# philgzl/brever

Measured on AMD Instinct MI355X. Metric: utterances/sec (4 s @16 kHz) Conv-TasNet train, higher is better.
Workload: dtype bf16

## Files before the change

### brever_amd/csrc/bwd_fused.cuh

```cuda
#pragma once
#include "tcn_kernels.cuh"

namespace brv {

#ifndef BF_ABL
#define BF_ABL 0
#endif

#ifndef BF_AHEAD1
#define BF_AHEAD1 4
#endif
#ifndef BF_AHEAD2
#define BF_AHEAD2 4
#endif
#ifndef BF_PIPE
#define BF_PIPE 1
#endif

struct BwdFusedParams {
  DwParams d;
  const bf16_t* g;
  int ldg, Kg;
  const bf16_t* Wp;
  const float* gamma2;
  float* dgamma2; float* dbeta2;
  int K, R;
#ifdef BF_STAMP
  long long* dbg;
#endif
};

#ifndef BF_ROWS_N
#define BF_ROWS_N 256
#endif
#ifndef BF_WPS
#define BF_WPS 3
#endif
constexpr int BF_ROWS = BF_ROWS_N;
constexpr int BF_LDW = HL_CG + 8;
constexpr int BF_LDS = BF_ROWS*BF_LDW*2 + 32*HL_CG*4;

inline void bf_tile_shape(int T, int dil, int P, int& K, int& R) {
  const int n_teeth = (T - 1)/dil + 1;
  long long best = -1;
  K = 1; R = 1;
  for (int r = 1; r <= HL_RMAX*2 && r <= dil; ++r) {
    const int kmax = BF_ROWS/r - (P - 1);
    if (kmax < 1) break;
    const int n_qt = ceil_div(n_teeth, kmax);
    const int k = ceil_div(n_teeth, n_qt);
    const long long tiles = (long long)n_qt*ceil_div(dil, r);
    const long long cost = tiles*100000 + tiles*(k + P - 1)*r;
    if (best < 0 || cost <= best) { best = cost; K = k; R = r; }
  }
}

#ifdef BF_STAMP
#define BF_MARK(i) do { long long t_; asm volatile("s_memtime %0\n\ts_waitcnt lgkmcnt(0)" : "=s"(t_) :: "memory"); \
                        if (threadIdx.x == 0 && fp.dbg) fp.dbg[(long long)blockIdx.x*8 + (i)] = t_; } while (0)
#else
#define BF_MARK(i) do { } while (0)
#endif
constexpr int kRowBad = 1 << 21;
constexpr int kRowCentre = 1 << 30;
constexpr int kRowFrame = kRowCentre - 1;
inline bool bf_frames_ok(long long T) { return T < kRowBad; }

template <int P, int KG>
__global__ __launch_bounds__(256, BF_WPS) void dwconv_bwd_fused_kernel(const BwdFusedParams fp) {
  const DwParams& p = fp.d;
  extern __shared__ __attribute__((aligned(16))) unsigned char dyn_lds[];
  bf16_t* win = reinterpret_cast<bf16_t*>(dyn_lds);
  float* red = reinterpret_cast<float*>(dyn_lds + BF_ROWS*BF_LDW*2);
  const int tid = threadIdx.x, lane = tid & 63, wid = tid >> 6;
  const int T = p.T, d = p.dil;
  const int R = fp.R, K = fp.K;
  const int n_rt = ceil_div(d, R);
  const int n_teeth = (T - 1)/d + 1;
  const int n_qt = ceil_div(n_teeth, K);
  const int n_tt = n_rt*n_qt, n_cg = p.Cp/HL_CG;
  const int xcd = blockIdx.x & 7, slot = blockIdx.x >> 3;
  const int cg = slot % n_cg;
  const int id = (slot / n_cg)*8 + xcd;
  if (id >= n_tt*p.B) return;
  const int b = id / n_tt;
  const int tile = id % n_tt;
  const int r0 = (tile % n_rt)*R, q0 = (tile / n_rt)*K;
  BF_MARK(0);
  const int cl = (tid & 7)*8;
  const int c0 = cg*HL_CG + cl;
  const int rslot = tid >> 3;
  const int W = (K + P - 1)*R;
  const int KR = K*R;
  const int qbase = q0 - (P - 1) + p.left/d;
  __shared__ int wtab[BF_ROWS];
  __shared__ int otab[BF_ROWS];
  {
    int qi, ri;
    if ((R & (R - 1)) == 0) { ri = tid & (R - 1); qi = tid >> (31 - __builtin_clz(R)); }
    else {
      qi = (int)(((float)tid + 0.5f)*(1.f/(float)R)); ri = tid - qi*R;
    }
    const int q = qbase + qi;
    const int tf = q*d + r0 + ri;
    const bool in = tid < W && q >= 0 && r0 + ri < d && tf < T;
    wtab[tid] = in ? (tf | ((q >= q0 && q < q0 + K) ? kRowCentre : 0)) : kRowBad;
    const int to = (q0 + qi)*d + r0 + ri;
    otab[tid] = (tid < KR && r0 + ri < d && to < T) ? to : kRowBad;
  }
  __shared__ float ptab[(3 + P)*HL_CG];
  float pv0 = 0.f, pv1 = 0.f;
  auto ptab_src = [&](int idx) -> const float* {
    const int which = idx >> 6, c = cg*HL_CG + (idx & 63);
    return which == 0 ? fp.gamma2 + c : which == 1 ? p.gamma1 + c : which == 2 ? p.beta1 + c
                      : p.taps + (long long)c*P + (which - 3);
  };
  {
    const float* s0 = ptab_src(tid);
    if (s0) pv0 = *s0;
    if (tid + 256 < (3 + P)*HL_CG) { const float* s1 = ptab_src(tid + 256); if (s1) pv1 = *s1; }
  }
  asm volatile("s_waitcnt lgkmcnt(0)\n\ts_barrier" ::: "memory");

  const __amdgpu_buffer_rsrc_t rz2 = make_rsrc(p.z2in + (long long)b*T*p.Cp, (long long)T*p.Cp*2);
  const __amdgpu_buffer_rsrc_t rz1 = make_rsrc(p.z1 + (long long)b*T*p.Cp, (long long)T*p.Cp*2);
  const unsigned int row = (unsigned int)(p.Cp*2), coff = (unsigned int)(c0*2);
  auto row_off = [&](int v) { return __umul24((unsigned int)(v & kRowFrame), row) + coff; };
  uint4 qzA[4], qz1A[4];
  {
    const int n32 = lane & 31, h = lane >> 5;
    const int oct = lane & 7, rsub = lane >> 3;
    const int widu = __builtin_amdgcn_readfirstlane(wid);
    const int ngrp = (W + 31) >> 5;
    const bool act0 = 2*widu < ngrp, act1 = 2*widu + 1 < ngrp;
    const __amdgpu_buffer_rsrc_t rg =
        make_rsrc(fp.g + (long long)b*T*fp.ldg, ((long long)(T - 1)*fp.ldg + KG)*2);
    unsigned int offG[8];
#pragma unroll
    for (int i = 0; i < 8; ++i)
      offG[i] = __umul24((unsigned int)(wtab[64*widu + 8*i + rsub] & kRowFrame), (unsigned int)(fp.ldg*2)) + (unsigned int)(oct*16);
    constexpr int nkc = KG >> 6;
    const bf16_t* wsrc0 = fp.Wp + (long long)(cg*2)*32*KG + lane*8;
    const bf16_t* wsrc1 = wsrc0 + (long long)32*KG;
    const uint4 z4 = make_uint4(0, 0, 0, 0);
    uint4 gq0 = z4, gq1 = z4, gq2 = z4, gq3 = z4, gq4 = z4, gq5 = z4, gq6 = z4, gq7 = z4;
    auto gl = [&](int i, int kc) { return buf_load16(rg, offG[i] + (unsigned int)(kc*128)); };
    auto gload = [&](int kc) {
      gq0 = gl(0, kc); gq1 = gl(1, kc); gq2 = gl(2, kc); gq3 = gl(3, kc);
      gq4 = gl(4, kc); gq5 = gl(5, kc); gq6 = gl(6, kc); gq7 = gl(7, kc);
    };
    bf16_t* gp = win + (64*widu + rsub)*BF_LDW + oct*8;
    auto gstore = [&]() {
      *reinterpret_cast<uint4*>(gp) = gq0;
      *reinterpret_cast<uint4*>(gp + 8*BF_LDW) = gq1;
      *reinterpret_cast<uint4*>(gp + 16*BF_LDW) = gq2;
      *reinterpret_cast<uint4*>(gp + 24*BF_LDW) = gq3;
      *reinterpret_cast<uint4*>(gp + 32*BF_LDW) = gq4;
      *reinterpret_cast<uint4*>(gp + 40*BF_LDW) = gq5;
      *reinterpret_cast<uint4*>(gp + 48*BF_LDW) = gq6;
      *reinterpret_cast<uint4*>(gp + 56*BF_LDW) = gq7;
    };
    bf16x8 a0_0, a0_1, a0_2, a0_3, a1_0, a1_1, a1_2, a1_3;
    auto al = [&](const bf16_t* w, int kc, int s) {
      return *reinterpret_cast<const bf16x8*>(w + kc*2048 + s*512);
    };
    f32x16 acc[2][2];
#pragma unroll
    for (int q = 0; q < 2; ++q)
#pragma unroll
      for (int ms = 0; ms < 2; ++ms)
#pragma unroll
        for (int i = 0; i < 16; ++i) acc[q][ms][i] = 0.f;
    const bf16_t* brow = win + (64*widu + n32)*BF_LDW + h*8;
    auto step = [&](int s, const bf16x8& a0, const bf16x8& a1) {
      if (BF_ABL & 1) return;
      if (act0) {
        const bf16x8 bv = *reinterpret_cast<const bf16x8*>(brow + s*16);
        acc[0][0] = __builtin_amdgcn_mfma_f32_32x32x16_bf16(a0, bv, acc[0][0], 0, 0, 0);
        acc[0][1] = __builtin_amdgcn_mfma_f32_32x32x16_bf16(a1, bv, acc[0][1], 0, 0, 0);
      }
      if (act1) {
        const bf16x8 bv = *reinterpret_cast<const bf16x8*>(brow + 32*BF_LDW + s*16);
        acc[1][0] = __builtin_amdgcn_mfma_f32_32x32x16_bf16(a0, bv, acc[1][0], 0, 0, 0);
        acc[1][1] = __builtin_amdgcn_mfma_f32_32x32x16_bf16(a1, bv, acc[1][1], 0, 0, 0);
      }
    };
    if (act0 && !(BF_ABL & 4)) {
      if (!(BF_ABL & 2)) {
        gload(0);
        a0_0 = al(wsrc0, 0, 0); a1_0 = al(wsrc1, 0, 0); a0_1 = al(wsrc0, 0, 1); a1_1 = al(wsrc1, 0, 1);
        a0_2 = al(wsrc0, 0, 2); a1_2 = al(wsrc1, 0, 2); a0_3 = al(wsrc0, 0, 3); a1_3 = al(wsrc1, 0, 3);
      }
#pragma unroll
      for (int kc = 0; kc < nkc; ++kc) {
        gstore();
        const bool more = kc + 1 < nkc && !(BF_ABL & 2);
        if (more) gload(kc + 1);
        step(0, a0_0, a1_0);
        if (more) { a0_0 = al(wsrc0, kc + 1, 0); a1_0 = al(wsrc1, kc + 1, 0); }
        step(1, a0_1, a1_1);
        if (more) { a0_1 = al(wsrc0, kc + 1, 1); a1_1 = al(wsrc1, kc + 1, 1); }
        step(2, a0_2, a1_2);
        if (more) { a0_2 = al(wsrc0, kc + 1, 2); a1_2 = al(wsrc1, kc + 1, 2); }
        step(3, a0_3, a1_3);
        if (more) { a0_3 = al(wsrc0, kc + 1, 3); a1_3 = al(wsrc1, kc + 1, 3); }
      }
    }
#pragma unroll
    for (int u = 0; u < 4; ++u) qzA[u] = buf_load16(rz2, row_off(wtab[rslot + 32*u]));
#pragma unroll
    for (int q = 0; q < 2; ++q) {
      if (!(q == 0 ? act0 : act1)) continue;
      const int wr = 64*widu + 32*q + n32;
#pragma unroll
      for (int ms = 0; ms < 2; ++ms)
#pragma unroll
        for (int gq = 0; gq < 4; ++gq) {
          uint2 v;
          v.x = pack2(acc[q][ms][4*gq], acc[q][ms][4*gq + 1]);
          v.y = pack2(acc[q][ms][4*gq + 2], acc[q][ms][4*gq + 3]);
          *reinterpret_cast<uint2*>(win + wr*BF_LDW + ms*32 + 8*gq + 4*h) = v;
        }
    }
  }
  BF_MARK(1);
  ptab[tid] = pv0;
  if (tid + 256 < (3 + P)*HL_CG) ptab[tid + 256] = pv1;
  __syncthreads();
  BF_MARK(2);

  const double mean2 = p.stats2[stat_sum(b)]*p.inv_n;
  double var2 = p.stats2[stat_sq(b)]*p.inv_n - mean2*mean2;
  if (var2 < 0.0) var2 = 0.0;
  const float rs2 = rstd_f32(var2 + (double)p.eps);
  const float mu2 = (float)mean2;
  const double S1 = p.sums2[stat_sum(b)], S2 = p.sums2[stat_sq(b)];
  const float m1 = (float)(S1*p.inv_n);
  const float m2 = rs2*(float)((S2 - mean2*S1)*p.inv_n);
  const float a2 = *p.slope2;
  const float c0s = 0.5f*(1.f + a2), c1s = 0.5f*(1.f - a2);
  const float ya = c0s*rs2, yb = c1s*rs2, yc = -mu2*rs2;
  const float R2 = rs2, K0 = -m1*rs2, M2R = -m2*rs2;
  f32x2 daz = {0.f, 0.f};
  f32x2 dbia[4], dgam2[4], dbet2[4], g2[4];
#pragma unroll
  for (int j = 0; j < 4; ++j) {
    g2[j] = f32x2{ptab[cl + 2*j], ptab[cl + 2*j + 1]};
    dbia[j] = f32x2{0.f, 0.f}; dgam2[j] = f32x2{0.f, 0.f}; dbet2[j] = f32x2{0.f, 0.f};
  }
  auto phase1_row = [&](int r, const uint4& qzv) {
      const int v = wtab[r];
      const float on = (v & kRowBad) ? 0.f : 1.f;
      const bool centre = v >= kRowCentre;
      const f32x2 rr = {on*R2, on*R2}, k0 = {on*K0, on*K0}, mm = {on*M2R, on*M2R};
      const f32x2 yav = {ya, ya}, ybv = {yb, yb}, ycv = {yc, yc}, c0v = {c0s, c0s}, c1v = {c1s, c1s};
      float e[8], z[8];
      unpack8(*reinterpret_cast<const uint4*>(win + r*BF_LDW + cl), e);
      unpack8(qzv, z);
      f32x2 gg[4], xg[4], ee[4], dd[4];
#pragma unroll
      for (int j = 0; j < 4; ++j) {
        const f32x2 zz = {z[2*j], z[2*j + 1]};
        ee[j] = f32x2{e[2*j], e[2*j + 1]};
        const f32x2 sg = {__uint_as_float((__float_as_uint(zz.x) & 0x80000000u) | 0x3f800000u),
                          __uint_as_float((__float_as_uint(zz.y) & 0x80000000u) | 0x3f800000u)};
        xg[j] = (yav + ybv*sg)*zz + ycv;
        const f32x2 uu = mm*xg[j] + ((ee[j]*g2[j])*rr + k0);
        const f32x2 us = uu*sg;
        gg[j] = c0v*uu + c1v*us;
        dd[j] = (uu - us)*zz;
      }
      uint4 q4;
      q4.x = pack2(gg[0].x, gg[0].y); q4.y = pack2(gg[1].x, gg[1].y);
      q4.z = pack2(gg[2].x, gg[2].y); q4.w = pack2(gg[3].x, gg[3].y);
      *reinterpret_cast<uint4*>(win + r*BF_LDW + cl) = q4;
      if (centre) {
#pragma unroll
        for (int j = 0; j < 4; ++j) {
          daz += dd[j];
          dbia[j] += gg[j];
          dgam2[j] += ee[j]*xg[j]; dbet2[j] += ee[j];
        }
      }
  };
  {
    uint4 qzB[4];
#pragma unroll
    for (int u = 0; u < 4; ++u) qzB[u] = buf_load16(rz2, row_off(wtab[rslot + 128 + 32*u]));
#pragma unroll
    for (int u = 0; u < 4; ++u) { const int r = rslot + 32*u; if (r < W) phase1_row(r, qzA[u]); }
#pragma unroll
    for (int u = 0; u < 4; ++u) qz1A[u] = buf_load16(rz1, row_off(otab[rslot + 32*u]));
#pragma unroll
    for (int u = 0; u < 4; ++u) { const int r = rslot + 128 + 32*u; if (r < W) phase1_row(r, qzB[u]); }
  }
  float da2 = 0.5f*(daz.x + daz.y);
  const int rep_off = id % kReplicas;
  auto swap32 = [](float& a, float& b) {
    const auto r = __builtin_amdgcn_permlane32_swap(__float_as_uint(a), __float_as_uint(b), false, false);
    a = __uint_as_float(r[0]); b = __uint_as_float(r[1]);
  };
  auto swap16 = [](float& a, float& b) {
    const auto r = __builtin_amdgcn_permlane16_swap(__float_as_uint(a), __float_as_uint(b), false, false);
    a = __uint_as_float(r[0]); b = __uint_as_float(r[1]);
  };
  auto ror8_add = [](float x) {
    return x + __int_as_float(__builtin_amdgcn_update_dpp(0, __float_as_int(x), 0x128, 0xf, 0xf, false));
  };
  auto fold8 = [&](const f32x2 (&v)[4], float& xa, float& xb) {
    float p[4], q[4];
#pragma unroll
    for (int j = 0; j < 4; ++j) { p[j] = v[j].x; q[j] = v[j].y; swap32(p[j], q[j]); p[j] += q[j]; }
    swap16(p[0], p[1]); xa = p[0] + p[1];
    swap16(p[2], p[3]); xb = p[2] + p[3];
    xa = ror8_add(xa); xb = ror8_add(xb);
  };
  const int fold_ch = (lane & 7)*8 + (((lane >> 4) & 1)*2 + (lane >> 5));
  auto put8 = [&](int vec, const f32x2 (&v)[4]) {
    float xa, xb;
    fold8(v, xa, xb);
    if (!(lane & 8)) {
      float* dst = red + (vec*4 + wid)*HL_CG + fold_ch;
      dst[0] = xa; dst[4] = xb;
    }
  };
  auto vec_sum = [&](int vec, int ch) {
    const float* src = red + vec*4*HL_CG + ch;
    return (src[0] + src[HL_CG]) + (src[2*HL_CG] + src[3*HL_CG]);
  };
  if (BF_ABL & 64) {
    float keep = da2;
#pragma unroll
    for (int j = 0; j < 4; ++j) keep += dbia[j].x*dbia[j].y + dgam2[j].x*dgam2[j].y + dbet2[j].x*dbet2[j].y;
    if (keep == 123.456f) red[tid] = keep;
  }
  if (!(BF_ABL & (16 | 64))) {
    da2 = wave_sum(da2);
    put8(0, dbia); put8(1, dgam2); put8(2, dbet2);
    if (lane == 0) red[3*4*HL_CG + wid] = da2;
    __syncthreads();
    if (tid < 3*HL_CG) {
      const int vec = tid >> 6, ch = tid & 63, c = cg*HL_CG + ch;
      float* dst = (vec == 0 ? p.dbias : vec == 1 ? fp.dgamma2 : fp.dbeta2) + (long long)rep_off*p.rep_stride;
      if (c < p.C && !(BF_ABL & 32)) atomic_add_f32(dst + c, vec_sum(vec, ch));
    } else if (tid == 3*HL_CG && !(BF_ABL & 32)) {
      const float* sc = red + 3*4*HL_CG;
      atomic_add_f32(p.dslope2 + (long long)rep_off*p.rep_stride, (sc[0] + sc[1]) + (sc[2] + sc[3]));
    }
  }
  __syncthreads();
  BF_MARK(4);

  const NormStat ns = norm_stat(p.stats1, b, p.inv_n, p.eps);
  const float a1 = *p.slope1;
  const float xa = 0.5f*(1.f + a1)*ns.rstd, xb = 0.5f*(1.f - a1)*ns.rstd, xc = -ns.mean*ns.rstd;
  f32x2 gm[4], be[4], w[P][4];
#pragma unroll
  for (int j = 0; j < 4; ++j) {
    gm[j] = f32x2{ptab[HL_CG + cl + 2*j], ptab[HL_CG + cl + 2*j + 1]};
    be[j] = f32x2{ptab[2*HL_CG + cl + 2*j], ptab[2*HL_CG + cl + 2*j + 1]};
#pragma unroll
    for (int k = 0; k < P; ++k)
      w[k][j] = f32x2{ptab[(3 + k)*HL_CG + cl + 2*j], ptab[(3 + k)*HL_CG + cl + 2*j + 1]};
  }
  f32x2 dgam[4], dbet[4], dtap[P][4];
#pragma unroll
  for (int j = 0; j < 4; ++j) {
    dgam[j] = f32x2{0.f, 0.f}; dbet[j] = f32x2{0.f, 0.f};
#pragma unroll
    for (int k = 0; k < P; ++k) dtap[k][j] = f32x2{0.f, 0.f};
  }
  const __amdgpu_buffer_rsrc_t re1 = make_rsrc(p.e1 + (long long)b*T*p.Cp, (long long)T*p.Cp*2);
  float l1 = 0.f, l2 = 0.f;
  auto phase2_row = [&](int i, const uint4& qz) {
    const int v = otab[i];
    if (v & kRowBad) return;
    float zc[8];
    unpack8(qz, zc);
    f32x2 xh[4], hn[4], dh[4];
#pragma unroll
    for (int j = 0; j < 4; ++j) {
      xh[j].x = __builtin_fmaf(xb, __builtin_fabsf(zc[2*j]), __builtin_fmaf(xa, zc[2*j], xc));
      xh[j].y = __builtin_fmaf(xb, __builtin_fabsf(zc[2*j + 1]), __builtin_fmaf(xa, zc[2*j + 1], xc));
      hn[j] = gm[j]*xh[j] + be[j];
      dh[j] = f32x2{0.f, 0.f};
    }
#pragma unroll
    for (int k = 0; k < P; ++k) {
      const int r = i + (P - 1 - k)*R;
      float g[8];
      unpack8(*reinterpret_cast<const uint4*>(win + r*BF_LDW + cl), g);
#pragma unroll
      for (int j = 0; j < 4; ++j) {
        const f32x2 gk = {g[2*j], g[2*j + 1]};
        dh[j] += w[k][j]*gk;
        dtap[k][j] += gk*hn[j];
      }
    }
    f32x2 o[4];
#pragma unroll
    for (int j = 0; j < 4; ++j) {
      const f32x2 dl = dh[j];
      o[j] = gm[j]*dl;
      dgam[j] += dl*xh[j]; dbet[j] += dl;
    }
    buf_store16(re1, __umul24((unsigned int)v, row) + coff, pack8v(o));
  };
  {
    uint4 qz1B[4];
#pragma unroll
    for (int u = 0; u < 4; ++u) qz1B[u] = buf_load16(rz1, row_off(otab[rslot + 128 + 32*u]));
#pragma unroll
    for (int u = 0; u < 4; ++u) { const int i = rslot + 32*u; if (i < KR) phase2_row(i, qz1A[u]); }
#pragma unroll
    for (int u = 0; u < 4; ++u) { const int i = rslot + 128 + 32*u; if (i < KR) phase2_row(i, qz1B[u]); }
  }
  BF_MARK(5);
#pragma unroll
  for (int j = 0; j < 4; ++j) {
    l1 += gm[j].x*dbet[j].x + gm[j].y*dbet[j].y;
    l2 += gm[j].x*dgam[j].x + gm[j].y*dgam[j].y;
  }

  if (BF_ABL & 64) {
    float keep = l1 + l2;
#pragma unroll
    for (int j = 0; j < 4; ++j) {
      keep += dgam[j].x*dgam[j].y + dbet[j].x*dbet[j].y;
#pragma unroll
      for (int k = 0; k < P; ++k) keep += dtap[k][j].x*dtap[k][j].y;
    }
    if (keep == 123.456f) red[tid] = keep;
  }
  if (!(BF_ABL & (16 | 64))) {
    l1 = wave_sum(l1); l2 = wave_sum(l2);
    put8(0, dgam); put8(1, dbet);
#pragma unroll
    for (int k = 0; k < P; ++k) put8(2 + k, dtap[k]);
    if (lane == 0) { red[(2 + P)*4*HL_CG + wid] = l1; red[(2 + P)*4*HL_CG + 4 + wid] = l2; }
    __syncthreads();
    for (int idx = tid; idx < (2 + P)*HL_CG; idx += 256) {
      const int vec = idx >> 6, ch = idx & 63, c = cg*HL_CG + ch;
      if (c >= p.C || (BF_ABL & 32)) continue;
      const float sum = vec_sum(vec, ch);
      if (vec == 0) atomic_add_f32(p.dgamma1 + (long long)rep_off*p.rep_stride + c, sum);
      else if (vec == 1) atomic_add_f32(p.dbeta1 + (long long)rep_off*p.rep_stride + c, sum);
      else atomic_add_f32(p.dtaps + (long long)rep_off*p.rep_stride + (long long)c*P + (vec - 2), sum);
    }
    if (tid == 255 && !(BF_ABL & 32)) {
      const float* sc = red + (2 + P)*4*HL_CG;
      atomic_add_f64(p.sums1 + stat_sum(b), ((double)sc[0] + (double)sc[1]) + ((double)sc[2] + (double)sc[3]));
      atomic_add_f64(p.sums1 + stat_sq(b), ((double)sc[4] + (double)sc[5]) + ((double)sc[6] + (double)sc[7]));
    }
  }
  BF_MARK(6);
}

struct GuDotsParams {
  const bf16_t* g; int ldg; const bf16_t* u; int ldu; const float* v1; int ncols; int B, T;
  double* out;
};
__global__ __launch_bounds__(256) void gu_dots_kernel(const GuDotsParams p) {
  __shared__ double dscr[16];
  const int b = blockIdx.y, tid = threadIdx.x;
  const int cpr = p.ncols/8;
  const long long per_item = (long long)p.T*cpr;
  double s1 = 0.0, s2 = 0.0;
  for (long long i = (long long)blockIdx.x*256 + tid; i < per_item; i += (long long)gridDim.x*256) {
    const int c = (int)(i % cpr)*8; const long long t = i / cpr;
    float gv[8], uv[8];
    unpack8(*reinterpret_cast<const uint4*>(p.g + ((long long)b*p.T + t)*p.ldg + c), gv);
    unpack8(*reinterpret_cast<const uint4*>(p.u + ((long long)b*p.T + t)*p.ldu + c), uv);
    float a = 0.f, q = 0.f;
#pragma unroll
    for (int j = 0; j < 8; ++j) { a = __builtin_fmaf(gv[j], p.v1[c + j], a); q = __builtin_fmaf(gv[j], uv[j], q); }
    s1 += a; s2 += q;
  }
  const double r1 = block_sum(s1, dscr);
  const double r2 = block_sum(s2, dscr + 8);
  if (tid == 0) {
    atomic_add_f64(p.out + stat_sum(b), r1);
    atomic_add_f64(p.out + stat_sq(b), r2);
  }
}

}
```

### brever_amd/csrc/bwd_fused_p.cuh

```cuda
#pragma once
#include "bwd_fused.cuh"

namespace brv {

template <int P, int KG>
__global__ __launch_bounds__(256, BF_WPS) void dwconv_bwd_fused_p_kernel(const BwdFusedParams fp, const int NT) {
  const DwParams& p = fp.d;
  extern __shared__ __attribute__((aligned(16))) unsigned char dyn_lds[];
  bf16_t* win = reinterpret_cast<bf16_t*>(dyn_lds);
  float* red = reinterpret_cast<float*>(dyn_lds + BF_ROWS*BF_LDW*2);
  const int tid = threadIdx.x, lane = tid & 63, wid = tid >> 6;
  const int T = p.T, d = p.dil;
  const int R = fp.R, K = fp.K;
  const float invR = 1.f/(float)R;
  const bool r_pow2 = (R & (R - 1)) == 0;
  const int lgR = 31 - __builtin_clz(R);
  auto divR = [&](int r, int& rem) {
    if (r_pow2) { rem = r & (R - 1); return r >> lgR; }
    const int q = (int)(((float)r + 0.5f)*invR);
    rem = r - q*R;
    return q;
  };
  const int n_rt = ceil_div(d, R);
  const int n_teeth = (T - 1)/d + 1;
  const int n_qt = ceil_div(n_teeth, K);
  const int n_tt = n_rt*n_qt, n_cg = p.Cp/HL_CG;
  const int xcd = blockIdx.x & 7, slot = blockIdx.x >> 3;
  const int cg = slot % n_cg;
  const int id0 = (slot / n_cg)*NT*8 + xcd;
  if (id0 >= n_tt*p.B) return;
  __shared__ float ptab[(3 + P)*HL_CG];
  {
    for (int idx = tid; idx < (3 + P)*HL_CG; idx += 256) {
      const int which = idx >> 6, c = cg*HL_CG + (idx & 63);
      ptab[idx] = which == 0 ? fp.gamma2[c] : which == 1 ? p.gamma1[c] : which == 2 ? p.beta1[c]
                             : p.taps[(long long)c*P + (which - 3)];
    }
    for (int idx = tid; idx < 32*HL_CG; idx += 256) red[idx] = 0.f;
  }
  const int rep_off = id0 % kReplicas;
  float da2_run = 0.f, l1_run = 0.f, l2_run = 0.f;
  int sum_item = -1;
  auto flush_item = [&]() {
    if (sum_item < 0) return;
    const float s1 = wave_sum(l1_run), s2 = wave_sum(l2_run);
    if (lane == 0 && !(BF_ABL & 32)) {
      atomic_add_f64(p.sums1 + stat_sum(sum_item), (double)s1);
      atomic_add_f64(p.sums1 + stat_sq(sum_item), (double)s2);
    }
    l1_run = 0.f; l2_run = 0.f;
  };
#pragma unroll 1
  for (int kt = 0; kt < NT; ++kt) {
  const int id = id0 + kt*8;
  if (id >= n_tt*p.B) break;
  int tv_ = threadIdx.x;
  asm volatile("" : "+v"(tv_));
  const int tid = tv_, lane = tid & 63, wid = tid >> 6;
  const int cl = (tid & 7)*8;
  const int c0 = cg*HL_CG + cl;
  const int rslot = tid >> 3;
  const int b = id / n_tt;
  const int tile = id % n_tt;
  const int r0 = (tile % n_rt)*R, q0 = (tile / n_rt)*K;
  if (b != sum_item) { flush_item(); sum_item = b; }
  if (kt > 0) __syncthreads();
  BF_MARK(0);
  const int W = (K + P - 1)*R;
  const int KR = K*R;
  const int qbase = q0 - (P - 1) + p.left/d;
  auto frame_of = [&](int r, bool& ok) {
    int ri;
    const int qi = divR(r, ri);
    const int q = qbase + qi;
    ok = r < W && q >= 0 && r0 + ri < d;
    return q*d + r0 + ri;
  };

  const __amdgpu_buffer_rsrc_t rz2 = make_rsrc(p.z2in + (long long)b*T*p.Cp, (long long)T*p.Cp*2);
  const unsigned int row = (unsigned int)(p.Cp*2), coff = (unsigned int)(c0*2);
  uint4 qzA[4];
  const __amdgpu_buffer_rsrc_t rz1 = make_rsrc(p.z1 + (long long)b*T*p.Cp, (long long)T*p.Cp*2);
  uint4 qz1A[4];
  auto out_frame = [&](int i, bool& ok) {
    int ri;
    const int qi = divR(i, ri);
    const int ro = r0 + ri;
    ok = i < KR && ro < d;
    return (q0 + qi)*d + ro;
// ... 382 lines not shown
```

### brever_amd/csrc/convtasnet.hip

```cpp
#include <hip/hip_runtime.h>
#include <stdio.h>
#include <stdlib.h>
#include <string.h>
#include <algorithm>
#include <string>
#include <vector>

#include "../../include/brever_hip.h"
#include "gemm_rows.cuh"
#include "gemm_wgrad.cuh"
#include "gemm_ws.cuh"
#include "dwpw2_fused.cuh"
#ifdef BRV_WITH_VARIANTS
#include "dwpw2_fused_v2.cuh"
#else
constexpr int D2_TT = 64;
#endif
#include "gemm_wgrad_full.cuh"
#include "gemm_wgrad_full128.cuh"

constexpr int kWgSplit = 4;
#include "prep.cuh"
#include "tcn_kernels.cuh"
#include "bwd_fused.cuh"
// ... 370 lines not shown
  const WgradParams& p = gp.base;
  if (p.T <= 0 || p.B <= 0) return 0;
  const int nprob = gp.nprob > 0 ? gp.nprob : 1;
  ProfScope prof(label, 2.0*nprob*p.B*p.T*(double)p.Gp*p.Hp, bytes*nprob, st);
  if (p.Hp % 64 != 0) return fail(-1, "wgrad: unpadded dims");
  const int target = wgrad_target(label, target_dflt);
  if (p.Hp % 128 == 0) return launch_wgrad_t<128, HK>(gp, st, target);
  return launch_wgrad_t<64, HK>(gp, st, target);
}
template <int HK>
int launch_wgrad(WgradParams& p, hipStream_t st, const char* label = "wgrad",
                 double bytes = 0, int target_dflt = 384) {
  WgradGroupParams gp;
  gp.base = p; gp.nprob = 0;
  return launch_wgrad_group<HK>(gp, st, label, bytes, target_dflt);
}

template <template <int> class F, typename... Args>
int dispatch_p(int P, Args&&... args) {
  switch (P) {
    case 1: return F<1>::run(args...);
    case 2: return F<2>::run(args...);
    case 3: return F<3>::run(args...);
    case 4: return F<4>::run(args...);
    case 5: return F<5>::run(args...);
  }
  return fail(-2, "unsupported kernel_size");
}
template <int P> struct DwFwd {
  static int run(const DwParams& p, hipStream_t st) {
    ProfScope prof("dwconv_fwd", 2.0*P*p.B*p.T*(double)p.Cp, 4.0*p.B*p.T*(double)p.Cp, st);
    dim3 grid(ceil_div(p.T, DW_TT_F)*p.B);
    hipLaunchKernelGGL((dwconv_fwd_kernel<P>), grid, dim3(256), 0, st, p);
    HIP_OK(hipGetLastError());
    return 0;
  }
};
template <int P> struct DwBwd {
  static int run(const DwParams& p, hipStream_t st) {
    if (p.z2in != nullptr) {
      static const char* by_dil[9] = {"dwconv_bwd_d1", "dwconv_bwd_d2", "dwconv_bwd_d4", "dwconv_bwd_d8", "dwconv_bwd_d16",
                                      "dwconv_bwd_d32", "dwconv_bwd_d64", "dwconv_bwd_d128", "dwconv_bwd_dx"};
      int lg = 0; while ((1 << lg) < p.dil && lg < 8) ++lg;
      ProfScope prof(prof_by_dil() ? by_dil[lg] : "dwconv_bwd", 4.0*P*p.B*p.T*(double)p.Cp, 8.0*p.B*p.T*(double)p.Cp, st);
      const int R = hl_rows_per_tooth(p.dil), K = HL_TT/R;
      const int tiles = ceil_div(p.dil, R)*ceil_div((p.T - 1)/p.dil + 1, K);
      dim3 grid(tiles*p.B*(p.Cp/HL_CG));
      const size_t lds = (size_t)hl_window_rows(p.dil, P)*HL_CG*2;
      hipLaunchKernelGGL((dwconv_bwd_halo_kernel<P>), grid, dim3(256), lds, st, p);
      HIP_OK(hipGetLastError());
      return 0;
    }
    ProfScope prof("dwconv_bwd", 4.0*P*p.B*p.T*(double)p.Cp, 6.0*p.B*p.T*(double)p.Cp, st);
    dim3 grid(ceil_div(p.T, DW_TT_B)*p.B);
    hipLaunchKernelGGL((dwconv_bwd_kernel<P>), grid, dim3(256), 0, st, p);
    HIP_OK(hipGetLastError());
    return 0;
  }
};

template <int P> struct DwBwdFused {
  static int run(const BwdFusedParams& p0, hipStream_t st) {
    BwdFusedParams p = p0;
    const DwParams& d = p.d;
#ifdef BF_STAMP
    p.dbg = debug_buffer();
#endif
    bf_tile_shape(d.T, d.dil, P, p.K, p.R);
    const int tiles = ceil_div(d.dil, p.R)*ceil_div((d.T - 1)/d.dil + 1, p.K);
    static const char* by_dil[9] = {"dwpw2_bwd_d1", "dwpw2_bwd_d2", "dwpw2_bwd_d4", "dwpw2_bwd_d8", "dwpw2_bwd_d16",
                                    "dwpw2_bwd_d32", "dwpw2_bwd_d64", "dwpw2_bwd_d128", "dwpw2_bwd_dx"};
    int lg = 0; while ((1 << lg) < d.dil && lg < 8) ++lg;
    ProfScope prof(prof_by_dil() ? by_dil[lg] : "dwpw2_bwd", 2.0*d.B*d.T*(double)d.Cp*(p.Kg + 2*P),
                   2.0*d.B*d.T*((double)p.Kg + 3.0*d.Cp), st);
    dim3 grid(ceil_div(tiles*d.B, 8)*8*(d.Cp/HL_CG));
    if (d.C != d.Cp) return fail(-1, "fused backward: channel count must be a multiple of 64");
#ifndef BF_NT
#define BF_NT 2
#endif
    const int nt = opt(BRV_OPT_BWD_PERSIST) ? BF_NT : 1;
    if (nt > 1 && p.Kg == 256) {
#ifdef BRV_WITH_VARIANTS
      dim3 gridp(ceil_div(ceil_div(tiles*d.B, 8), nt)*8*(d.Cp/HL_CG));
      hipLaunchKernelGGL((dwconv_bwd_fused_p_kernel<P, 256>), gridp, dim3(256), BF_LDS, st, p, nt);
#else
      return fail(-1, "BRV_OPT_BWD_PERSIST: the persistent fused backward is not in this build (tools/mkvariant.sh <tag> -DBRV_WITH_VARIANTS)");
#endif
    } else
    if (p.Kg == 256) hipLaunchKernelGGL((dwconv_bwd_fused_kernel<P, 256>), grid, dim3(256), BF_LDS, st, p);
    else if (p.Kg == 128) hipLaunchKernelGGL((dwconv_bwd_fused_kernel<P, 128>), grid, dim3(256), BF_LDS, st, p);
    else return fail(-1, "fused backward: unexpected [res | skip] width");
    HIP_OK(hipGetLastError());
    return 0;
  }
};

int launch_dz(const DzParams& p, hipStream_t st) {
  ProfScope prof("gln_prelu_bwd", 0, 6.0*p.B*p.T*(double)p.Cp, st);
  const long long per_item = (long long)p.T*(p.Cp/8);
  int gx = (int)((per_item + 256*8 - 1)/(256*8));
  const int cap = 1024/p.B > 1 ? 1024/p.B : 1;
  if (gx > cap) gx = cap;
  if (gx < 1) gx = 1;
  hipLaunchKernelGGL(dz_kernel, dim3(gx, p.B), dim3(256), 0, st, p);
  HIP_OK(hipGetLastError());
  return 0;
}

ASpec rows_bf16(const void* ptr, int ld, long long T) {
  ASpec a; memset(&a, 0, sizeof(a));
  a.p0 = ptr; a.ld0 = ld; a.bs0 = T*ld; a.K0 = 1 << 30; a.nsrc = 1;
  return a;
}
void set_affine(ASpec& a, const double* stats, const float* g, const float* b, int C,
                long long T) {
  a.stats = stats; a.gamma = g; a.beta = b; a.C = C;
  a.inv_n = 1.0/((double)T*(double)C); a.eps = 1e-8f;
}
ASpec frames_of(const float* wav, long long L, int hop, int K, long long stride = 0) {
  ASpec a; memset(&a, 0, sizeof(a));
  a.p0 = wav; a.hop = hop; a.Kf = K; a.wav_stride = stride > 0 ? stride : L; a.wav_len = (int)L;
  a.K0 = 1 << 30; a.nsrc = 1;
  return a;
}

struct PrepJobC { int src_off, dst_off, scale_off; unsigned short R, C, rows, cols, dst_ld, tr; };
constexpr int kPrepBatch = 168;
struct PrepBatch { PrepJobC jobs[kPrepBatch]; int n; };
static_assert(sizeof(PrepBatch) <= 4096, "kernel argument size");

struct PackJob { long long src_off, dst_off; int N, K, nsl; };
struct PackBatch { PackJob jobs[96]; int n; };
__global__ __launch_bounds__(256) void pack_frag_kernel(bf16_t* prepared, const PackBatch pb) {
  const PackJob j = pb.jobs[blockIdx.y];
  const long long total = (long long)j.N*j.K/8;
  const int KS = j.K/16;
  for (long long i = (long long)blockIdx.x*256 + threadIdx.x; i < total; i += (long long)gridDim.x*256) {
    const int n = (int)(i / (j.K/8)), k = (int)(i % (j.K/8))*8;
    const int slice = n / j.nsl, f = (n % j.nsl)/32, fr = n % 32, s = k/16, fh = (k % 16)/8;
    const long long dst = (long long)slice*j.nsl*j.K + ((long long)(f*KS + s)*64 + fr + 32*fh)*8;
    *reinterpret_cast<uint4*>(prepared + j.dst_off + dst) =
        *reinterpret_cast<const uint4*>(prepared + j.src_off + (long long)n*j.K + k);
  }
}
__global__ __launch_bounds__(256) void prep_weights_kernel(const float* params,
                                                           bf16_t* prepped,
                                                           const PrepBatch pb) {
  const PrepJobC& c = pb.jobs[blockIdx.y];
  PrepJob j;
  j.src_off = c.src_off; j.dst_off = c.dst_off; j.scale_off = c.scale_off;
  j.R = c.R; j.C = c.C; j.rows = c.rows; j.cols = c.cols; j.dst_ld = c.dst_ld; j.tr = c.tr;
  prep_job_run(params, prepped, j, blockIdx.x, gridDim.x);
}

struct LazyPrepBlk { long long res_w, res_b, skip_w, skip_b, beta, wg, out; };
struct LazyPrepParams {
  int nb, H, Hp, Bn, Sc, Bnp, Scp;
  int* stamp; int stamp_value;
  LazyPrepBlk blk[kWgMaxProb];
};
__global__ __launch_bounds__(256) void lazy_prep_kernel(const float* params, bf16_t* prepped,
                                                        const LazyPrepParams p) {
  const LazyPrepBlk& b = p.blk[blockIdx.y];
  float* out = reinterpret_cast<float*>(prepped + b.out);
  const int NP = p.Bnp + p.Scp;
  const int n = blockIdx.x*4 + (threadIdx.x >> 6), lane = threadIdx.x & 63;
  if (blockIdx.x == 0 && blockIdx.y == 0 && threadIdx.x == 0) *p.stamp = p.stamp_value;
// ... 1221 lines not shown
```

Measured before the change: 2454.

## Stream gradient tiles into an LDS ring via direct buffer-to-LDS loads in fused backward

The pointwise-GEMM prologue of the fused depthwise backward kernel no longer stages g rows through registers and then stores them to the LDS window. It issues buffer_load...lds directly into a per-wave ring of GRING slots, using an XOR swizzle and vmcnt-counted waits, so MFMA stages overlap with later loads. The reduction scratch is folded into the LDS window padding to shrink the LDS footprint, and the z2/z1 row prefetch becomes double-buffered batches of configurable depth. Risks are the subtle vmcnt accounting and extra barriers when the ring aliases the window.

```diff
diff --git a/brever_amd/csrc/bwd_fused.cuh b/brever_amd/csrc/bwd_fused.cuh
--- a/brever_amd/csrc/bwd_fused.cuh
+++ b/brever_amd/csrc/bwd_fused.cuh
@@ -1,5 +1,7 @@
 #pragma once
+#include <type_traits>
 #include "tcn_kernels.cuh"
+#include "gemm_wgrad_full.cuh"
 
 namespace brv {
 
@@ -15,6 +17,9 @@
 #endif
 #ifndef BF_PIPE
 #define BF_PIPE 1
+#endif
+#ifndef BF_GRING
+#define BF_GRING 3
 #endif
 
 struct BwdFusedParams {
@@ -36,9 +41,27 @@
 #ifndef BF_WPS
 #define BF_WPS 3
 #endif
+#ifndef BF_WPS_P
+#define BF_WPS_P 3
+#endif
 constexpr int BF_ROWS = BF_ROWS_N;
 constexpr int BF_LDW = HL_CG + 8;
-constexpr int BF_LDS = BF_ROWS*BF_LDW*2 + 32*HL_CG*4;
+constexpr int BF_RING = BF_GRING*4096;
+constexpr int BF_LDS = BF_ROWS*BF_LDW*2 > 4*BF_RING ? BF_ROWS*BF_LDW*2 : 4*BF_RING;
+constexpr int BF_LDS_P = BF_ROWS*BF_LDW*2 + 32*HL_CG*4;
+
+constexpr int bf_younger(int st, int nr, int nt) {
+  int y = 0;
+  for (int u = st + 1; u <= st + nr - 1 && u < nt; ++u) y += u % 2 == 0 ? 12 : 4;
+  return y;
+}
+
+template <class F, int... I>
+__device__ __forceinline__ void static_for_(F&& f, std::integer_sequence<int, I...>) {
+  (f(std::integral_constant<int, I>{}), ...);
+}
+template <int N, class F>
+__device__ __forceinline__ void static_for(F&& f) { static_for_(f, std::make_integer_sequence<int, N>{}); }
 
 inline void bf_tile_shape(int T, int dil, int P, int& K, int& R) {
   const int n_teeth = (T - 1)/dil + 1;
@@ -71,7 +94,10 @@
   const DwParams& p = fp.d;
   extern __shared__ __attribute__((aligned(16))) unsigned char dyn_lds[];
   bf16_t* win = reinterpret_cast<bf16_t*>(dyn_lds);
-  float* red = reinterpret_cast<float*>(dyn_lds + BF_ROWS*BF_LDW*2);
+  float* red = reinterpret_cast<float*>(dyn_lds);
+  auto bf_pad = [&](int i) -> float* {
+    return reinterpret_cast<float*>(dyn_lds + (i >> 2)*(BF_LDW*2) + HL_CG*2) + (i & 3);
+  };
   const int tid = threadIdx.x, lane = tid & 63, wid = tid >> 6;
   const int T = p.T, d = p.dil;
   const int R = fp.R, K = fp.K;
@@ -126,43 +152,51 @@
   const __amdgpu_buffer_rsrc_t rz1 = make_rsrc(p.z1 + (long long)b*T*p.Cp, (long long)T*p.Cp*2);
   const unsigned int row = (unsigned int)(p.Cp*2), coff = (unsigned int)(c0*2);
   auto row_off = [&](int v) { return __umul24((unsigned int)(v & kRowFrame), row) + coff; };
-  uint4 qzA[4], qz1A[4];
+  constexpr int N1 = BF_AHEAD1, N2 = BF_AHEAD2;
+  static_assert(8 % N1 == 0 && 8 % N2 == 0, "batches of rows");
+  uint4 qz[2][N1], qz1[2][N2];
   {
     const int n32 = lane & 31, h = lane >> 5;
-    const int oct = lane & 7, rsub = lane >> 3;
     const int widu = __builtin_amdgcn_readfirstlane(wid);
     const int ngrp = (W + 31) >> 5;
     const bool act0 = 2*widu < ngrp, act1 = 2*widu + 1 < ngrp;
     const __amdgpu_buffer_rsrc_t rg =
         make_rsrc(fp.g + (long long)b*T*fp.ldg, ((long long)(T - 1)*fp.ldg + KG)*2);
-    unsigned int offG[8];
-#pragma unroll
-    for (int i = 0; i < 8; ++i)
-      offG[i] = __umul24((unsigned int)(wtab[64*widu + 8*i + rsub] & kRowFrame), (unsigned int)(fp.ldg*2)) + (unsigned int)(oct*16);
-    constexpr int nkc = KG >> 6;
+    constexpr int NC = KG >> 6, NT = 2*NC;
+    constexpr int NR = BF_GRING, SLOT = 4096;
+    static_assert(NR >= 2 && 4*BF_RING + (2*BF_ROWS + (3 + P)*HL_CG)*4 <= 160*1024/3, "three workgroups per CU");
+    unsigned char* ring = dyn_lds + widu*BF_RING;
+    constexpr bool ring_shared = BF_RING > 64*BF_LDW*2;
+    unsigned int offG[2][4];
+#pragma unroll
+    for (int q = 0; q < 2; ++q)
+#pragma unroll
+      for (int j = 0; j < 4; ++j) {
+        const int r = 8*j + (lane >> 3);
+        offG[q][j] = __umul24((unsigned int)(wtab[64*widu + 32*q + r] & kRowFrame), (unsigned int)(fp.ldg*2))
+                   + (unsigned int)((((lane & 7) ^ ((r >> 1) & 7)))*16);
+      }
+    unsigned int rb[4];
+#pragma unroll
+    for (int s = 0; s < 4; ++s) rb[s] = lds_addr(ring) + (unsigned int)(n32*128 + (((2*s + h) ^ ((n32 >> 1) & 7)))*16);
     const bf16_t* wsrc0 = fp.Wp + (long long)(cg*2)*32*KG + lane*8;
     const bf16_t* wsrc1 = wsrc0 + (long long)32*KG;
-    const uint4 z4 = make_uint4(0, 0, 0, 0);
-    uint4 gq0 = z4, gq1 = z4, gq2 = z4, gq3 = z4, gq4 = z4, gq5 = z4, gq6 = z4, gq7 = z4;
-    auto gl = [&](int i, int kc) { return buf_load16(rg, offG[i] + (unsigned int)(kc*128)); };
-    auto gload = [&](int kc) {
-      gq0 = gl(0, kc); gq1 = gl(1, kc); gq2 = gl(2, kc); gq3 = gl(3, kc);
-      gq4 = gl(4, kc); gq5 = gl(5, kc); gq6 = gl(6, kc); gq7 = gl(7, kc);
-    };
-    bf16_t* gp = win + (64*widu + rsub)*BF_LDW + oct*8;
-    auto gstore = [&]() {
-      *reinterpret_cast<uint4*>(gp) = gq0;
-      *reinterpret_cast<uint4*>(gp + 8*BF_LDW) = gq1;
-      *reinterpret_cast<uint4*>(gp + 16*BF_LDW) = gq2;
-      *reinterpret_cast<uint4*>(gp + 24*BF_LDW) = gq3;
-      *reinterpret_cast<uint4*>(gp + 32*BF_LDW) = gq4;
-      *reinterpret_cast<uint4*>(gp + 40*BF_LDW) = gq5;
-      *reinterpret_cast<uint4*>(gp + 48*BF_LDW) = gq6;
-      *reinterpret_cast<uint4*>(gp + 56*BF_LDW) = gq7;
-    };
-    bf16x8 a0_0, a0_1, a0_2, a0_3, a1_0, a1_1, a1_2, a1_3;
-    auto al = [&](const bf16_t* w, int kc, int s) {
-      return *reinterpret_cast<const bf16x8*>(w + kc*2048 + s*512);
+    bf16x8 a0[2][4], a1[2][4];
+    auto issue = [&](auto tc) {
+      constexpr int ST = decltype(tc)::value, c = ST/2, q = ST % 2;
+      if (BF_ABL & 2) return;
+      if constexpr (q == 0) {
+#pragma unroll
+        for (int s = 0; s < 4; ++s) {
+          a0[c % 2][s] = *reinterpret_cast<const bf16x8*>(wsrc0 + (4*c + s)*512);
+          a1[c % 2][s] = *reinterpret_cast<const bf16x8*>(wsrc1 + (4*c + s)*512);
+        }
+      }
+      unsigned char* dst = ring + (ST % NR)*SLOT;
+#pragma unroll
+      for (int j = 0; j < 4; ++j)
+        __builtin_amdgcn_raw_ptr_buffer_load_lds(rg, (lds_void_p)(dst + 1024*j), 16, (int)offG[q][j], c*128, 0, 0);
+      __builtin_amdgcn_sched_barrier(0);
     };
     f32x16 acc[2][2];
 #pragma unroll
@@ -171,43 +205,32 @@
       for (int ms = 0; ms < 2; ++ms)
 #pragma unroll
         for (int i = 0; i < 16; ++i) acc[q][ms][i] = 0.f;
-    const bf16_t* brow = win + (64*widu + n32)*BF_LDW + h*8;
-    auto step = [&](int s, const bf16x8& a0, const bf16x8& a1) {
+    auto stage = [&](auto tc) {
+      constexpr int ST = decltype(tc)::value, c = ST/2, q = ST % 2;
+      if constexpr (ST + NR - 1 < NT) issue(std::integral_constant<int, ST + NR - 1>{});
+      asm volatile("s_waitcnt vmcnt(%0)" :: "n"(bf_younger(ST, NR, NT)) : "memory");
+      u32x4 bv[4];
+#pragma unroll
+      for (int s = 0; s < 4; ++s)
+        asm volatile("ds_read_b128 %0, %1 offset:%2" : "=v"(bv[s]) : "v"(rb[s]), "n"((ST % NR)*SLOT) : "memory");
+      lds_wait16(bv[0], bv[1]);
+      lds_wait16(bv[2], bv[3]);
       if (BF_ABL & 1) return;
-      if (act0) {
-        const bf16x8 bv = *reinterpret_cast<const bf16x8*>(brow + s*16);
-        acc[0][0] = __builtin_amdgcn_mfma_f32_32x32x16_bf16(a0, bv, acc[0][0], 0, 0, 0);
-        acc[0][1] = __builtin_amdgcn_mfma_f32_32x32x16_bf16(a1, bv, acc[0][1], 0, 0, 0);
-      }
-      if (act1) {
-        const bf16x8 bv = *reinterpret_cast<const bf16x8*>(brow + 32*BF_LDW + s*16);
-        acc[1][0] = __builtin_amdgcn_mfma_f32_32x32x16_bf16(a0, bv, acc[1][0], 0, 0, 0);
-        acc[1][1] = __builtin_amdgcn_mfma_f32_32x32x16_bf16(a1, bv, acc[1][1], 0, 0, 0);
+      if (!(q == 0 ? act0 : act1)) return;
+#pragma unroll
+      for (int s = 0; s < 4; ++s) {
+        const bf16x8 b = __builtin_bit_cast(bf16x8, bv[s]);
+        acc[q][0] = __builtin_amdgcn_mfma_f32_32x32x16_bf16(a0[c % 2][s], b, acc[q][0], 0, 0, 0);
+        acc[q][1] = __builtin_amdgcn_mfma_f32_32x32x16_bf16(a1[c % 2][s], b, acc[q][1], 0, 0, 0);
       }
     };
     if (act0 && !(BF_ABL & 4)) {
-      if (!(BF_ABL & 2)) {
-        gload(0);
-        a0_0 = al(wsrc0, 0, 0); a1_0 = al(wsrc1, 0, 0); a0_1 = al(wsrc0, 0, 1); a1_1 = al(wsrc1, 0, 1);
-        a0_2 = al(wsrc0, 0, 2); a1_2 = al(wsrc1, 0, 2); a0_3 = al(wsrc0, 0, 3); a1_3 = al(wsrc1, 0, 3);
-      }
-#pragma unroll
-      for (int kc = 0; kc < nkc; ++kc) {
-        gstore();
-        const bool more = kc + 1 < nkc && !(BF_ABL & 2);
-        if (more) gload(kc + 1);
-        step(0, a0_0, a1_0);
-        if (more) { a0_0 = al(wsrc0, kc + 1, 0); a1_0 = al(wsrc1, kc + 1, 0); }
-        step(1, a0_1, a1_1);
-        if (more) { a0_1 = al(wsrc0, kc + 1, 1); a1_1 = al(wsrc1, kc + 1, 1); }
-        step(2, a0_2, a1_2);
-        if (more) { a0_2 = al(wsrc0, kc + 1, 2); a1_2 = al(wsrc1, kc + 1, 2); }
-        step(3, a0_3, a1_3);
-        if (more) { a0_3 = al(wsrc0, kc + 1, 3); a1_3 = al(wsrc1, kc + 1, 3); }
-      }
-    }
-#pragma unroll
-    for (int u = 0; u < 4; ++u) qzA[u] = buf_load16(rz2, row_off(wtab[rslot + 32*u]));
+      static_for<NR - 1 < NT ? NR - 1 : NT>(issue);
+      static_for<NT>(stage);
+    }
+#pragma unroll
+    for (int u = 0; u < N1; ++u) qz[0][u] = buf_load16(rz2, row_off(wtab[rslot + 32*u]));
+    if constexpr (ring_shared) asm volatile("s_barrier" ::: "memory");
 #pragma unroll
     for (int q = 0; q < 2; ++q) {
       if (!(q == 0 ? act0 : act1)) continue;
@@ -283,16 +306,17 @@
         }
       }
   };
-  {
-    uint4 qzB[4];
-#pragma unroll
-    for (int u = 0; u < 4; ++u) qzB[u] = buf_load16(rz2, row_off(wtab[rslot + 128 + 32*u]));
-#pragma unroll
-    for (int u = 0; u < 4; ++u) { const int r = rslot + 32*u; if (r < W) phase1_row(r, qzA[u]); }
-#pragma unroll
-    for (int u = 0; u < 4; ++u) qz1A[u] = buf_load16(rz1, row_off(otab[rslot + 32*u]));
-#pragma unroll
-    for (int u = 0; u < 4; ++u) { const int r = rslot + 128 + 32*u; if (r < W) phase1_row(r, qzB[u]); }
+#pragma unroll
+  for (int k = 0; k < 8/N1; ++k) {
+    if (k + 1 < 8/N1) {
+#pragma unroll
+      for (int u = 0; u < N1; ++u) qz[(k + 1) & 1][u] = buf_load16(rz2, row_off(wtab[rslot + 32*(N1*(k + 1) + u)]));
+    } else {
+#pragma unroll
+      for (int u = 0; u < N2; ++u) qz1[0][u] = buf_load16(rz1, row_off(otab[rslot + 32*u]));
+    }
+#pragma unroll
+    for (int u = 0; u < N1; ++u) { const int r = rslot + 32*(N1*k + u); if (r < W) phase1_row(r, qz[k & 1][u]); }
   }
   float da2 = 0.5f*(daz.x + daz.y);
   const int rep_off = id % kReplicas;
@@ -316,36 +340,38 @@
     xa = ror8_add(xa); xb = ror8_add(xb);
   };
   const int fold_ch = (lane & 7)*8 + (((lane >> 4) & 1)*2 + (lane >> 5));
-  auto put8 = [&](int vec, const f32x2 (&v)[4]) {
+  auto scr = [&](bool pad, int i) -> float* { return pad ? bf_pad(i) : red + i; };
+  auto put8 = [&](bool pad, int vec, const f32x2 (&v)[4]) {
     float xa, xb;
     fold8(v, xa, xb);
     if (!(lane & 8)) {
-      float* dst = red + (vec*4 + wid)*HL_CG + fold_ch;
-      dst[0] = xa; dst[4] = xb;
-    }
-  };
-  auto vec_sum = [&](int vec, int ch) {
-    const float* src = red + vec*4*HL_CG + ch;
-    return (src[0] + src[HL_CG]) + (src[2*HL_CG] + src[3*HL_CG]);
+      const int i = (vec*4 + wid)*HL_CG + fold_ch;
+      *scr(pad, i) = xa; *scr(pad, i + 4) = xb;
+    }
+  };
+  auto vec_sum = [&](bool pad, int vec, int ch) {
+    const int i = vec*4*HL_CG + ch;
+    return (*scr(pad, i) + *scr(pad, i + HL_CG)) + (*scr(pad, i + 2*HL_CG) + *scr(pad, i + 3*HL_CG));
   };
   if (BF_ABL & 64) {
     float keep = da2;
 #pragma unroll
     for (int j = 0; j < 4; ++j) keep += dbia[j].x*dbia[j].y + dgam2[j].x*dgam2[j].y + dbet2[j].x*dbet2[j].y;
-    if (keep == 123.456f) red[tid] = keep;
+    if (keep == 123.456f) *bf_pad(tid) = keep;
   }
   if (!(BF_ABL & (16 | 64))) {
     da2 = wave_sum(da2);
-    put8(0, dbia); put8(1, dgam2); put8(2, dbet2);
-    if (lane == 0) red[3*4*HL_CG + wid] = da2;
+    put8(true, 0, dbia); put8(true, 1, dgam2); put8(true, 2, dbet2);
+    if (lane == 0) *bf_pad(3*4*HL_CG + wid) = da2;
     __syncthreads();
     if (tid < 3*HL_CG) {
       const int vec = tid >> 6, ch = tid & 63, c = cg*HL_CG + ch;
       float* dst = (vec == 0 ? p.dbias : vec == 1 ? fp.dgamma2 : fp.dbeta2) + (long long)rep_off*p.rep_stride;
-      if (c < p.C && !(BF_ABL & 32)) atomic_add_f32(dst + c, vec_sum(vec, ch));
+      if (c < p.C && !(BF_ABL & 32)) atomic_add_f32(dst + c, vec_sum(true, vec, ch));
     } else if (tid == 3*HL_CG && !(BF_ABL & 32)) {
-      const float* sc = red + 3*4*HL_CG;
-      atomic_add_f32(p.dslope2 + (long long)rep_off*p.rep_stride, (sc[0] + sc[1]) + (sc[2] + sc[3]));
+      const int i = 3*4*HL_CG;
+      atomic_add_f32(p.dslope2 + (long long)rep_off*p.rep_stride,
+                     (*bf_pad(i) + *bf_pad(i + 1)) + (*bf_pad(i + 2) + *bf_pad(i + 3)));
     }
   }
   __syncthreads();
@@ -406,14 +432,14 @@
     }
     buf_store16(re1, __umul24((unsigned int)v, row) + coff, pack8v(o));
   };
-  {
-    uint4 qz1B[4];
-#pragma unroll
-    for (int u = 0; u < 4; ++u) qz1B[u] = buf_load16(rz1, row_off(otab[rslot + 128 + 32*u]));
-#pragma unroll
-    for (int u = 0; u < 4; ++u) { const int i = rslot + 32*u; if (i < KR) phase2_row(i, qz1A[u]); }
-#pragma unroll
-    for (int u = 0; u < 4; ++u) { const int i = rslot + 128 + 32*u; if (i < KR) phase2_row(i, qz1B[u]); }
+#pragma unroll
+  for (int k = 0; k < 8/N2; ++k) {
+    if (k + 1 < 8/N2) {
+#pragma unroll
+      for (int u = 0; u < N2; ++u) qz1[(k + 1) & 1][u] = buf_load16(rz1, row_off(otab[rslot + 32*(N2*(k + 1) + u)]));
+    }
+#pragma unroll
+    for (int u = 0; u < N2; ++u) { const int i = rslot + 32*(N2*k + u); if (i < KR) phase2_row(i, qz1[k & 1][u]); }
   }
   BF_MARK(5);
 #pragma unroll
@@ -434,15 +460,16 @@
   }
   if (!(BF_ABL & (16 | 64))) {
     l1 = wave_sum(l1); l2 = wave_sum(l2);
-    put8(0, dgam); put8(1, dbet);
-#pragma unroll
-    for (int k = 0; k < P; ++k) put8(2 + k, dtap[k]);
+    __syncthreads();
+    put8(false, 0, dgam); put8(false, 1, dbet);
+#pragma unroll
+    for (int k = 0; k < P; ++k) put8(false, 2 + k, dtap[k]);
     if (lane == 0) { red[(2 + P)*4*HL_CG + wid] = l1; red[(2 + P)*4*HL_CG + 4 + wid] = l2; }
     __syncthreads();
     for (int idx = tid; idx < (2 + P)*HL_CG; idx += 256) {
       const int vec = idx >> 6, ch = idx & 63, c = cg*HL_CG + ch;
       if (c >= p.C || (BF_ABL & 32)) continue;
-      const float sum = vec_sum(vec, ch);
+      const float sum = vec_sum(false, vec, ch);
       if (vec == 0) atomic_add_f32(p.dgamma1 + (long long)rep_off*p.rep_stride + c, sum);
       else if (vec == 1) atomic_add_f32(p.dbeta1 + (long long)rep_off*p.rep_stride + c, sum);
       else atomic_add_f32(p.dtaps + (long long)rep_off*p.rep_stride + (long long)c*P + (vec - 2), sum);
diff --git a/brever_amd/csrc/bwd_fused_p.cuh b/brever_amd/csrc/bwd_fused_p.cuh
--- a/brever_amd/csrc/bwd_fused_p.cuh
+++ b/brever_amd/csrc/bwd_fused_p.cuh
@@ -4,7 +4,7 @@
 namespace brv {
 
 template <int P, int KG>
-__global__ __launch_bounds__(256, BF_WPS) void dwconv_bwd_fused_p_kernel(const BwdFusedParams fp, const int NT) {
+__global__ __launch_bounds__(256, BF_WPS_P) void dwconv_bwd_fused_p_kernel(const BwdFusedParams fp, const int NT) {
   const DwParams& p = fp.d;
   extern __shared__ __attribute__((aligned(16))) unsigned char dyn_lds[];
   bf16_t* win = reinterpret_cast<bf16_t*>(dyn_lds);
diff --git a/brever_amd/csrc/convtasnet.hip b/brever_amd/csrc/convtasnet.hip
--- a/brever_amd/csrc/convtasnet.hip
+++ b/brever_amd/csrc/convtasnet.hip
@@ -476,7 +476,7 @@
     if (nt > 1 && p.Kg == 256) {
 #ifdef BRV_WITH_VARIANTS
       dim3 gridp(ceil_div(ceil_div(tiles*d.B, 8), nt)*8*(d.Cp/HL_CG));
-      hipLaunchKernelGGL((dwconv_bwd_fused_p_kernel<P, 256>), gridp, dim3(256), BF_LDS, st, p, nt);
+      hipLaunchKernelGGL((dwconv_bwd_fused_p_kernel<P, 256>), gridp, dim3(256), BF_LDS_P, st, p, nt);
 #else
       return fail(-1, "BRV_OPT_BWD_PERSIST: the persistent fused backward is not in this build (tools/mkvariant.sh <tag> -DBRV_WITH_VARIANTS)");
 #endif
```

New measurement: 2452, median of 6. No clear change (-0.1%).
